# mitsuba-renderer/mitsuba2

Hardware: AMD Instinct MI355X
Metric: Msamples/sec (whole node), 1080p/512spp path integrator (higher is better)
Workload: dtype f32

## Files before the change

mitsuba2_amd/csrc/device/resident_kernel.h:

```cpp
#ifndef MIW_KERNEL
#define MIW_KERNEL __global__
#endif
MIW_KERNEL __launch_bounds__(MIW_BLOCK) void k_init_pixels(RenderParams P, U4 *st_out, uint32_t *pixel_out, InitArgs A) {
    uint32_t lane = blockIdx.x * blockDim.x + threadIdx.x;
    if (lane >= P.n_lanes) return;
    uint32_t tile = lane >> A.bs2_log2, i = lane & ((1u << A.bs2_log2) - 1u);
    uint32_t b = A.tile_list ? A.tile_list[tile] : tile;
    uint32_t bx = b % A.blocks_x, by = b / A.blocks_x;
    uint32_t x, y;
    morton_decode2(i, x, y);
    int32_t bw = P.film.crop_w - (int32_t) (bx * A.bs), bh = P.film.crop_h - (int32_t) (by * A.bs);
    if (bw > (int32_t) A.bs) bw = (int32_t) A.bs;
    if (bh > (int32_t) A.bs) bh = (int32_t) A.bs;
    if ((int32_t) x >= bw || (int32_t) y >= bh) {
        U4 st; st.x = st.y = 0; st.z = LF_DONE; st.w = 0;
        st_out[lane] = st; pixel_out[lane] = 0;
        return;
    }
    uint32_t px = (uint32_t) P.film.crop_x + bx * A.bs + x, py = (uint32_t) P.film.crop_y + by * A.bs + y;
    pixel_out[lane] = px | (py << 16);
    st_out[lane] = lane_seed_state(A.base_seed + (uint64_t) A.block_ids[b] * (uint64_t) (A.bs * A.bs) + i);
}

struct TileArgs {
    const uint32_t *tile_list; uint32_t blocks_x, bs, bs2_log2;
// ... 4 lines not shown
#ifndef MIW_PLACE_PIECES
#define MIW_PLACE_PIECES 4
#endif
template <bool Placed = true, bool Clock = false, bool Groups = false, bool Jobs = true, bool Frame = false>
struct QueueWork {
    static_assert(!Frame || (!Placed && !Groups && Jobs), "the frame twin: one queue of chunk jobs, no group counts");
    const LaneQueues *Q; uint32_t *next_pixel; uint32_t n_lanes, spp, lane, warn_negative;
    const FilmRec *film; const float *thr;
    uint32_t nq, per, q, dry, t_fetch;
    __device__ __forceinline__ void init_queues(uint32_t queues) {
        nq = Placed ? queues : 1u; per = nq > 1u ? MIW_PLACE_PIECES * 64u : n_lanes; q = 0u; dry = 0; t_fetch = 0;
        ticks = 0; quarter = 0; tail_prio = 0; sample_end_ = spp;
        if (Jobs) job_pend() = 0u;
        if (Placed && Q->simd_ids) {
            const uint32_t hw = (uint32_t) __builtin_amdgcn_s_getreg(4 | (0 << 6) | (31 << 11)),
                           xcc = (uint32_t) __builtin_amdgcn_s_getreg(20 | (0 << 6) | (3 << 11));
            const uint32_t key = ((xcc & 15u) << 10) | (((hw >> 13) & 7u) << 7) | (((hw >> 12) & 1u) << 6) | (((hw >> 8) & 15u) << 2) | ((hw >> 4) & 3u);
            if (nq > 1u) { const uint32_t id = Q->simd_ids[1u + key]; q = id < nq ? id : key % nq; }
            else if ((threadIdx.x & 63u) == 0u) Q->simd_ids[1u + key] = 1u;
        }
    }
    uint32_t ticks, quarter, tail_prio, sample_end_; uint32_t *prog;
    __device__ __forceinline__ void tick(uint32_t sample_idx, bool has_pixel) {
        if (Frame) return;
        if (!tail_prio) { ++ticks; return; }
        if ((uint32_t) __builtin_amdgcn_readfirstlane((int) ++ticks) & 15u) return;
        if (has_pixel) atomicMin(prog, sample_idx);
        const uint32_t v = *prog;
        *prog = 0xffffffffu;
        const uint32_t v4 = 4u * v, se = sample_end_;
        uint32_t qtr = v == 0xffffffffu ? 3u : (v4 >= se ? 1u : 0u) + (v4 >= 2u * se ? 1u : 0u) + (v4 >= 3u * se ? 1u : 0u);
        qtr = (uint32_t) __builtin_amdgcn_readfirstlane((int) qtr);
        if (qtr == quarter) return;
        quarter = qtr;
        if (qtr == 0u) __builtin_amdgcn_s_setprio(3); else if (qtr == 1u) __builtin_amdgcn_s_setprio(2);
        else if (qtr == 2u) __builtin_amdgcn_s_setprio(1); else __builtin_amdgcn_s_setprio(0);
    }
    __device__ __forceinline__ void enable_tail_prio(uint32_t sample_end, uint32_t *wave_word) {
        tail_prio = 1u; sample_end_ = sample_end; quarter = 0; prog = wave_word; *prog = 0xffffffffu; __builtin_amdgcn_s_setprio(3);
    }
    typedef uint32_t U4v __attribute__((ext_vector_type(4)));
    __device__ __forceinline__ static uint32_t &job_pend() { __shared__ uint32_t s_job_pend[MIW_BLOCK]; return s_job_pend[threadIdx.x & (MIW_BLOCK - 1)]; }
    __device__ __forceinline__ bool exhausted() const { return (!Frame && (!Jobs || !Q->job_chunk)) || job_pend() == 0xffffffffu; }
    __device__ __forceinline__ uint32_t job_end(uint32_t sample_idx, uint32_t sample_end) const {
        const uint32_t r = spp - sample_idx;
        return Jobs && (r & (r - 1u)) == 0u && r >= Q->job_min ? sample_idx : sample_end;
    }
    __device__ __forceinline__ bool fetch_job(uint32_t &pixel, U4 &st) {
        for (;;) {
            const uint32_t parked = job_pend();
            if (parked == 0xffffffffu) return false;
            uint32_t id = parked - 1u;
            const bool fresh = parked == 0u;
            const unsigned long long b = __ballot(fresh);
            if (fresh) {
                const uint32_t me = threadIdx.x & 63u, leader = (uint32_t) __ffsll((long long) b) - 1u;
                uint32_t base = 0;
                if (me == leader) base = atomicAdd(next_pixel, (uint32_t) __popcll(b));
                base = (uint32_t) __shfl((int) base, (int) leader, 64);
                id = base + __builtin_amdgcn_mbcnt_hi((uint32_t) (b >> 32), __builtin_amdgcn_mbcnt_lo((uint32_t) b, 0u));
                if (id >= Q->job_total) { job_pend() = 0xffffffffu; return false; }
            }
            const uint32_t j = id / n_lanes, slot = id - j * n_lanes;
            const uint32_t px = Q->pixel[slot];
            U4v w;
#if defined(__HIP_DEVICE_COMPILE__)
            asm volatile("global_load_dwordx4 %0, %1, off sc1\n\ts_waitcnt vmcnt(0)" : "=&v"(w) : "v"(Q->st + slot) : "memory");
#endif
            if (w.z & LF_DONE) { job_pend() = 0u; continue; }
            if (w.w != (j ? spp - (Q->job_pow >> (j - 1u)) : 0u)) { job_pend() = id + 1u; return false; }
            job_pend() = 0u;
            lane = slot; pixel = px;
            st.x = w.x; st.y = w.y; st.z = w.z; st.w = w.w;
            return true;
        }
    }
    __device__ __forceinline__ bool fetch(uint32_t &pixel, U4 &st) {
        if (Frame || (Jobs && Q->job_chunk)) return fetch_job(pixel, st);
        for (;;) {
            if (!Placed) {
                const unsigned long long b = __ballot(1);
                const uint32_t me = threadIdx.x & 63u, leader = (uint32_t) __ffsll((long long) b) - 1u;
                uint32_t base = 0;
                if (me == leader) base = atomicAdd(next_pixel, (uint32_t) __popcll(b));
                base = (uint32_t) __shfl((int) base, (int) leader, 64);
                const uint32_t l = base + __builtin_amdgcn_mbcnt_hi((uint32_t) (b >> 32), __builtin_amdgcn_mbcnt_lo((uint32_t) b, 0u));
                if (l >= n_lanes) return false;
                lane = l;
                st = Q->st[lane];
                if (st.z & LF_DONE) continue;
                pixel = Q->pixel[lane];
                return true;
            }
// ... 40 lines not shown
        }
        Q->st[lane] = st;
        if (Placed && Q->lane_cost) Q->lane_cost[lane] = cost_clock() - t_fetch + 1u;
        if (Groups && Q->group_done && (st.z & LF_DONE)) {
            __threadfence();
            const uint32_t g = lane >> Q->group_shift;
            if (atomicAdd(Q->group_done + g, 1u) + 1u == Q->group_expected[g]) {
                __threadfence_system();
                __hip_atomic_store(Q->group_flag + g, 1u, __ATOMIC_RELEASE, __HIP_MEMORY_SCOPE_SYSTEM);
            }
        }
    }
    __device__ __forceinline__ void put(uint32_t pixel, uint32_t sample_idx, V2 pos, const float *aovs) {
        if (Frame || Q->log_rec) {
            LogSink16<const float *> sink{ Q->log_rec, thr, film, lane, spp, Q->log_rej & 255u, Q->log_rej >> 8 };
            sink(pixel, sample_idx, pos, aovs);
        } else {
            LogSink sink; sink.log_pos = Q->log_pos; sink.log_val = Q->log_val; sink.lane = lane; sink.spp = spp; sink.warn_negative = warn_negative;
            sink(0u, sample_idx, pos, aovs);
        }
    }
};

#ifndef MIW_DIRECT_WAVES
#define MIW_DIRECT_WAVES 3
#endif
#ifndef MIW_PACKET_WAVES_ALL
#define MIW_PACKET_WAVES_ALL 4
#endif
#ifndef MIW_PACKET_WAVES
#define MIW_PACKET_WAVES 5
#endif
template <bool UseLog, int Tiny, int Mats = MATS_ALL, bool Analytic = (Tiny == 0), uint32_t Integ = INTEG_PATH, bool Groups = false, int Waves = 0, uint32_t Feat = FEAT_ALL>
__global__ __launch_bounds__(MIW_BLOCK, Waves ? Waves : Integ == INTEG_DIRECT ? MIW_DIRECT_WAVES : Tiny ? ((Mats == MATS_DIFFUSE && !MIW_SPECTRAL) ? (Tiny == 2 ? MIW_PACKET_WAVES : 4) : MIW_PACKET_WAVES_ALL) : MIW_TREE_WAVES) void k_path_resident(RenderParams P, SceneView sc, LaneQueues Q, double *accum, Counters *cnt,
                                                               TraceLds cfg, uint32_t sample_end, TileArgs T, uint32_t *next_pixel) {
    constexpr bool Frame = (Feat & FEAT_FRAME) != 0;
    static_assert(!Frame || (UseLog && Tiny != 0 && !Analytic && Integ == INTEG_PATH && !Groups && Waves == 0 && Feat == FEAT_FRAME), "a frame twin is the twin of a lean packet kernel");
    extern __shared__ uint4 smem[];
    stage_to_lds(sc, cfg, smem);
    const float *thr = stage_thresholds(smem, cfg, UseLog && (Frame || Q.log_rec) ? Q.log_thr : nullptr);
    constexpr bool Frames = MIW_LDS_TABLES && UseLog && Tiny != 0 && Integ != INTEG_DIRECT;
#if MIW_LDS_TABLES
    if constexpr (UseLog && Tiny != 0) stage_tables<true, mats_lights(Mats), mats_full(Mats), Frames>(sc, cfg, smem);
#endif
#if defined(MIW_SECTION_PROFILE) && defined(__HIP_DEVICE_COMPILE__)
    if ((threadIdx.x & 63u) == 0) { unsigned long long *b_ = miw_sec_buf(); for (int i = 0; i < 15; ++i) b_[i] = 0; b_[15] = __builtin_amdgcn_s_memtime(); }
// ... 3 lines not shown
    int tile_x0 = 0, tile_y0 = 0;
    if (!UseLog && T.side) {
        const uint32_t lane0 = blockIdx.x * blockDim.x, t = lane0 >> T.bs2_log2, q0 = lane0 & ((1u << T.bs2_log2) - 1u);
        const uint32_t b = T.tile_list ? T.tile_list[t] : t;
        uint32_t qx, qy;
        morton_decode2(q0, qx, qy);
        const int margin = (int) (T.side - 16u) / 2;
        tile_x0 = (int) ((b % T.blocks_x) * T.bs + qx) - margin;
        tile_y0 = (int) ((b / T.blocks_x) * T.bs + qy) - margin;
        for (uint32_t i = threadIdx.x; i < T.side * T.side * MIW_FILM_CHANNELS; i += blockDim.x) tile[i] = 0.0;
        __syncthreads();
    }
    LaneCounters local; local.segments = local.samples = local.shadow_rays = 0;
    auto tr2 = [&](V3 o, float mint, V3 dE, float maxtE, bool hasE, V3 dS, float maxtS, bool hasS, F4 &hE, bool &occS) {
        trace2<Tiny, Analytic, Integ != INTEG_DIRECT, Frame>(sc, cfg, smem, o, mint, dE, maxtE, hasE, dS, maxtS, hasS, hE, occS);
    };
    if (UseLog) {
        QueueWork<Tiny != 0 && !Frame, false, Groups, true, Frame> work; work.Q = &Q; work.next_pixel = next_pixel; work.n_lanes = P.n_lanes; work.spp = P.spp; work.lane = 0; work.warn_negative = P.film.warn_negative;
        work.film = &P.film; work.thr = thr; work.init_queues(cfg.queues ? cfg.queues : 1u);
        if constexpr (!Frame) {
            __shared__ uint32_t s_prog[MIW_BLOCK / 64];
            if (cfg.tail_prio) work.enable_tail_prio(sample_end, &s_prog[threadIdx.x >> 6]);
        }
        if constexpr (Integ == INTEG_DIRECT) pixel_stream_render_direct<Mats, Analytic>(P, sc, sample_end, work, tr2, &local);
        else pixel_stream_render<Mats, Analytic, Frames, Feat & FEAT_ALL>(P, sc, sample_end, work, tr2, &local);
    } else if (lane < P.n_lanes) {
        U4 st = Q.st[lane];
        if (!(st.z & LF_DONE)) {
            const uint32_t pixel = Q.pixel[lane];
            if (T.side) {
                TileAdd add; add.tile = tile; add.x0 = tile_x0; add.y0 = tile_y0; add.side = (int) T.side;
                SplatXYSink<TileAdd> sink; sink.film = &P.film; sink.add = add;
                st = pixel_render<Integ, mats_nested(Mats) ? Mats : MATS_ALL>(P, sc, pixel, st, sample_end, tr2, sink, &local);
            } else {
                FilmAdd add; add.accum = accum;
                SplatSink<FilmAdd> sink; sink.film = &P.film; sink.add = add;
                st = pixel_render<Integ, mats_nested(Mats) ? Mats : MATS_ALL>(P, sc, pixel, st, sample_end, tr2, sink, &local);
            }
            Q.st[lane] = st;
        }
    }
    if (!UseLog && T.side) {
        __syncthreads();
        const int n = (int) (T.side * T.side);
        for (int i = (int) threadIdx.x; i < n * MIW_FILM_CHANNELS; i += (int) blockDim.x) {
            const double v = tile[i];
            if (v == 0.0) continue;
            const int texel = i / MIW_FILM_CHANNELS, k = i - texel * MIW_FILM_CHANNELS;
            const int fx = tile_x0 + texel % (int) T.side, fy = tile_y0 + texel / (int) T.side;
            unsafeAtomicAdd(accum + ((size_t) fy * P.film.crop_w + fx) * MIW_FILM_CHANNELS + k, v);
        }
    }
    unsigned long long a = wave_sum(local.segments), b = wave_sum(local.samples), c = wave_sum(local.shadow_rays);
    if ((threadIdx.x & 63) == 0) {
        Counters *shard = cnt + ((blockIdx.x * (MIW_BLOCK / 64) + (threadIdx.x >> 6)) & (MIW_CNT_SHARDS - 1));
        if (a) atomicAdd(&shard->segments, a);
        if (b) atomicAdd(&shard->samples, b);
        if (c) atomicAdd(&shard->shadow_rays, c);
#if defined(MIW_SECTION_PROFILE) && defined(__HIP_DEVICE_COMPILE__)
        { unsigned long long *b_ = miw_sec_buf(); for (int i = 0; i < 15; ++i) if (b_[i]) atomicAdd(&g_sections[i], b_[i]); }
#endif
    }
}
```

mitsuba2_amd/csrc/miwave.hip:

```cpp
#include <hip/hip_runtime.h>
#include <stdio.h>
#include <stdlib.h>
#include <string.h>
#include <stdarg.h>
#include <string>
#include <vector>
#include <chrono>
#include <atomic>
#include <cmath>
#include <map>
#include <string>
#include <algorithm>

#include "../../include/miwave.h"
#include "kernel_pick.h"
#if defined(MIW_CLASS_PART) || defined(MIW_AOV_UNIT)
#define MIW_KERNELS_ONLY 1
#endif
#if defined(MIW_SECTION_PROFILE)
__device__ unsigned long long g_sections[16];
#endif
#if defined(MIW_PHASE_STATS)
__device__ unsigned long long g_phase_stats[15];
#endif
// ... 116 lines not shown
    { "MIW_MAX_LEAF", "host SAH builder: triangles per leaf" },
    { "MIW_NO_STACK", "1: no LDS-stack walk (stackless BVH2 walk, wavefront plan)" },
    { "MIW_BVH4", "0: no 4-wide tree (the phase machine steps through the BVH2)" },
    { "MIW_BVH4_FAN", "2 | 3 | 4: widest node the 4-wide collapse may build" },
    { "MIW_BVH4_HOST", "1: the 4-wide tree is collapsed on the host from the read-back BVH2" },
    { "MIW_BVH8", "0: mi_bvh_build skips the 8-wide tree / mi_render keeps the 4-wide walk" },
    { "MIW_STACK8_FULL", "1: the 8-wide walk keeps the 16-entry LDS column instead of one entry per tree level" },
    { "MIW_ENV_TOP", "0: the environment warp's top levels are not staged in LDS" },
    { "MIW_PHASED", "0: tree scenes take the lock-step kernel instead of the phase machine" },
    { "MIW_PHASED_WAVES", "3 | 4: wavefronts per SIMD the phase machine is launched for" },
    { "MIW_TRIO", "0: MATS_PLAIN kernels where the MATS_TRIO class would do" },
    { "MIW_SHADE_VOTE", "num:den of the phase machine's shade vote" },
    { "MIW_LOOP_EXIT", "node:triangle hand-over ratios of the phase machine's walk loops" },
    { "MIW_POOLED", "1: tree scenes take k_path_pooled (walk jobs pooled across the workgroup; experimental, slower: DESIGN.md)" },
    { "MIW_POOL_SHAPE", "12x1 | 8x2: wavefronts per workgroup x pixels per lane of k_path_pooled" },
    { "MIW_POOL_VOTE", "shade_min:walk_min:node_min:tri_min:claim_min of k_path_pooled" },
    { "MIW_TAIL_PRIO", "0: no least-progress-first wave priorities; 1: also in a packet kernel's launch of chunk jobs, which runs without them by default (and then keeps its lean kernel instead of the frame twin)" },
    { "MIW_WG_PER_CU", "workgroups per CU of the packet kernels' persistent grid" },
    { "MIW_PLACE", "0: shards of about one pixel per lane skip the measuring launch + placed queues" },
    { "MIW_JOB_CHUNK", "smallest chunk of a full frame's pixel jobs, in samples (a power of two; default 64, the phase machine 32): the pixels' sample streams are cut into halving chunks drawn chunk-major from one queue; 0: a job = all the samples of a pixel" },
    { "MIW_JOB_CHUNK_FORCE", "1: chunk jobs whatever the frame's size (tests of the hand-over between lanes)" },
    { "MIW_LEAN", "0: a packet scene without environment map and vertex normals, rendered without the moment integrator, keeps the full path kernel instead of its lean twin (kernel_pick.h: packet_features)" },
    { "MIW_FRAME_TWIN", "0: a full frame of chunk jobs keeps the lean twin of its packet path kernel instead of the frame twin, which has the facts of such a launch compiled in (kernel_pick.h: frame_twin)" },
    { "MIW_PACKET_SHARD4", "0: a plain-diffuse packet job of at most four wavefronts of pixels per SIMD keeps the five-wavefront (96-register) kernel" },
    { "MIW_PLACE_MEASURE", "divisor: the measuring launch runs spp / divisor samples" },
    { "MIW_PLACE_SPREAD", "0 | 1: placed pieces = consecutive sorted lanes | one lane of every cost stratum" },
    { "MIW_STREAM", "0: plan 1 walks with one kernel per list slice instead of the persistent stream kernel" },
    { "MIW_FILM_LEGACY", "1: the 24-byte position log + k_film_blocks for every filter" },
    { "MIW_FILM_LANES", "0 | 1 | 2: k_film_lanes off / over the tile-interleaved log / over [lane][sample]" },
    { "MIW_FILM_CHAINS", "0: the replay over the tile-interleaved log runs k_film_lanes (a wavefront per block position) instead of k_film_chains (a wavefront per chain of positions of equal weight)" },
    { "MIW_FILM_CHAINS_U", "4 | 8: records in flight per lane of k_film_chains: 8 (the default) compiled for two wavefronts per SIMD, 4 for three" },
    { "MIW_FILM_QUADS", "0 | 24 | 28 | 42 | 44: k_film_quads group shape (0: off)" },
    { "MIW_FILM_COLUMNS", "0 | 42 | 44 | 82: k_film_columns group shape" },
    { "MIW_FILM_GROUP", "2 | 3 | 4: k_film_groups group shape" },
    { "MIW_FL_NT", "0: k_film_lanes reads the log with plain instead of streaming loads" },
    { "MIW_FILM_OVERLAP", "1: part of the film replay of a full Cornell-class frame is queued on three more streams beside the path kernel, sets of 64-tile groups each behind the flags their last pixels raise (default 0: measured +0 - 1 %); 2: without the waits (timing probe: the film is the previous frame's)" },
    { "MIW_FILM_OVERLAP_SET", "groups of 64 tiles per launch of that replay (default 4)" },
    { "MIW_FILM_OVERLAP_ROOM", "workgroups the path kernel's grid is short of filling the device while the replay runs beside it (default 32: one per CU on 32 CUs)" },
    { "MIW_FILM_OVERLAP_LEAN", "0: the launches of that replay are the 168-register kernel (default 1: the 128-register form)" },
    { "MIW_FILM_OVERLAP_BESIDE", "groups of 64 tiles replayed beside the path kernel; the rest in one launch after it (default: three quarters)" },
    { "MIW_FILM_OVERLAP_PRIO", "s_setprio of the replay wavefronts that run beside the path kernel, 0 .. 3 (default 0)" },
    { "MIW_FQ_U", "2 | 4 | 8: records per trip of k_film_quads" },
    { "MIW_RCCL", "0: mi_film_reduce never uses RCCL (device add)" },
    { "MIW_RCCL_FORCE", "1: mi_film_reduce takes the RCCL branch for one context too (tests)" }
};
struct Options {
// ... 1758 lines not shown
static bool out_of_time(const RenderFrame &F) {
    return F.cfg->timeout_s > 0.f &&
           std::chrono::duration<double>(std::chrono::steady_clock::now() - F.wall0).count() > F.cfg->timeout_s;
}
static SceneView view_over_tree8(const mi_ctx *c) {
    SceneView v = c->view;
    v.nodes8 = c->d_nodes8.p; v.tris = c->d_tris8.p; if (v.tri_vn) v.tri_vn = c->d_tri_vn8.p;
    return v;
}
static InitArgs init_args(const RenderFrame &F) {
    InitArgs A; A.block_ids = F.c->d_block_ids.p; A.tile_list = F.cfg->tile_list ? F.c->d_tile_list.p : nullptr;
    A.blocks_x = F.blocks_x; A.blocks_y = F.blocks_y; A.bs = F.bs; A.bs2_log2 = F.bs2_log2; A.base_seed = F.cfg->base_seed;
    return A;
}

struct PathRoute {
    bool direct, tiny;
    uint32_t n_simd, per_launch;
    bool phased, phased_placeable, phased8; int ph_waves;
    bool packet_shard4; uint32_t feat, res_waves;
    bool place; uint32_t measure_end, n_pieces;
    int overlap_mode; bool overlap;
    bool pooled;
};
static mi_status path_route(RenderFrame &F, const miw_pick::Facts &facts, const RenderLds &L, PathRoute &R) {
    mi_ctx *c = F.c; const mi_render_cfg *cfg = F.cfg; const Options &ropt = F.ropt; const FilmPlan &FP = F.FP;
    const int film_mode = FP.film_mode; const uint32_t n_lanes = F.n_lanes, n_tiles = F.n_tiles;
    const bool direct = F.P.integrator == INTEG_DIRECT, tables_fit = L.lay.tables_fit; const size_t rlds = L.lay.rlds;
    const uint32_t n_simd = (uint32_t) c->cu_count * 4u;
    const uint32_t per_launch = cfg->samples_per_launch > 0 ? (uint32_t) cfg->samples_per_launch : 128u;
    const bool tiny = facts.tiny;
    const bool phased_on = !ropt.off("MIW_PHASED");
    const bool trio_kernel = miw_pick::trio_kernel(facts);
    const bool phased = phased_on && !direct && !tiny && c->lds_cfg.stack && (c->view.nodes4 != nullptr || trio_kernel) && (tables_fit || !MIW_LDS_TABLES);
    const int ph_waves = ropt.num("MIW_PHASED_WAVES", 4) == 4 ? 4 : 3;
    const bool phased_placeable = phased && c->view.nodes4 != nullptr && ph_waves == 4;
    const bool phased8 = phased_placeable && L.walk8;
    if (L.stack8_sized && !phased8) return fail(c, MI_ERR_STATE, "render: the LDS stack was sized for the 8-wide walk, which this launch does not run");
    bool packet_shard4 = !phased && tiny && c->diffuse_only && !MIW_SPECTRAL && !direct && c->view.tri_count <= 32u && MIW_PACKET_WAVES > 4 && film_mode == 1 && n_lanes <= 64u * 4u * n_simd;
    if (ropt.off("MIW_PACKET_SHARD4")) packet_shard4 = false;
    const uint32_t feat = miw_pick::packet_features_kernel(miw_pick::packet_features(c->have_env, c->shape_normals, c->emitter_normals, cfg->moment_pass != 0), !ropt.off("MIW_LEAN"));
    const uint32_t res_waves_compiled = miw_plan::res_waves_compiled(phased, (uint32_t) ph_waves, tiny, c->diffuse_only && !MIW_SPECTRAL, c->view.tri_count <= 32u, packet_shard4,
                                                                     (uint32_t) MIW_TREE_WAVES, (uint32_t) MIW_PACKET_WAVES, (uint32_t) MIW_PACKET_WAVES_ALL);
    const uint32_t res_waves = tiny && film_mode == 1 ? std::max(1u, std::min(res_waves_compiled, miw_plan::lds_workgroups(rlds))) : res_waves_compiled;
    bool place = film_mode == 1 && !direct && (tiny || phased_placeable) && miw_plan::place_window(n_lanes, res_waves, n_simd) &&
                 cfg->spp >= 128u && per_launch >= cfg->spp && cfg->timeout_s <= 0.f;
    if (ropt.off("MIW_PLACE")) place = false;
    uint32_t measure_div = (uint32_t) std::max(2, ropt.num("MIW_PLACE_MEASURE", 8));
    const uint32_t measure_end = place ? std::max<uint32_t>(16u, cfg->spp / measure_div) : 0u;
    const uint32_t n_pieces = (n_lanes + 63u) / 64u;
    const int overlap_mode = ropt.num("MIW_FILM_OVERLAP", 0);
    const bool overlap = overlap_mode != 0 && c->overlap_state != 0 && film_mode == 1 && FP.rec16 && FP.film_lanes != 0 && FP.log_il != 0 && !place && !phased  && tiny && c->diffuse_only && !MIW_SPECTRAL && !direct  &&
                         per_launch >= cfg->spp && cfg->timeout_s <= 0.f && n_tiles > 0;
#if MIW_SPECTRAL
    const bool pooled = false;
#else
    const bool pooled = phased8 && !place && L.pooled_fits;
#endif
    R.direct = direct; R.tiny = tiny; R.n_simd = n_simd; R.per_launch = per_launch;
    R.phased = phased; R.phased_placeable = phased_placeable; R.phased8 = phased8; R.ph_waves = ph_waves;
    R.packet_shard4 = packet_shard4; R.feat = feat; R.res_waves = res_waves;
    R.place = place; R.measure_end = measure_end; R.n_pieces = n_pieces;
    R.overlap_mode = overlap_mode; R.overlap = overlap; R.pooled = pooled;
    return MI_OK;
}

static mi_status place_prepare(RenderFrame &F, const PathRoute &R, size_t &place_tmp_bytes) {
// ... 45 lines not shown
        HIP_TRY(c, hipStreamSynchronize(s));
        if (first_lane < n_lanes) HIP_TRY(c, hipMemcpy(&px, c->q_pixel.p + first_lane, sizeof(uint32_t), hipMemcpyDeviceToHost));
        double csum = 0.0; uint32_t with = 0;
        for (uint32_t v : all) if (v) { csum += (double) v; ++with; }
        K.place_cost_max = all.empty() ? 0u : all[0]; K.place_cost_mean = with ? csum / with : 0.0; K.place_max_pixel = px;
        K.place_cost_unit = phased ? 1u : 0u; K.place_measure_spp = measure_end;
    }
    if (K.placed && ropt.get("MIW_DEBUG")) {
        std::vector<uint32_t> cur(n_simd), ids(1u + (1u << 14)), cost(n_pieces);
        (void) hipMemcpy(cur.data(), c->d_next_pixel.p, n_simd * sizeof(uint32_t), hipMemcpyDeviceToHost);
        (void) hipMemcpy(ids.data(), c->d_simd_ids.p, ids.size() * sizeof(uint32_t), hipMemcpyDeviceToHost);
        (void) hipMemcpy2D(cost.data(), sizeof(uint32_t), c->d_cost_sorted.p, Q.piece_a * sizeof(uint32_t), sizeof(uint32_t), n_pieces, hipMemcpyDeviceToHost);
        uint32_t keys = 0, key_or = 0, full = 0, over = 0; uint64_t csum = 0; uint32_t cmin = ~0u, cmax = 0;
        for (uint32_t k = 0; k < (1u << 14); ++k) if (ids[1 + k] != 0xffffffffu) { ++keys; key_or |= k; }
        ids[0] = keys;
        for (uint32_t v : cur) { full += v >= 64u * MIW_PLACE_PIECES; over += v > 64u * MIW_PLACE_PIECES; }
        for (uint32_t v : cost) { csum += v; cmin = std::min(cmin, v); cmax = std::max(cmax, v); }
        fprintf(stderr, "[miwave] placed queues: %u SIMDs numbered, %u distinct hardware keys (bits used 0x%x), %u of %u queues drained (%u asked beyond their end), "
                        "cost of the dearest pixel of a piece min / mean / max = %u / %.0f / %u (iterations, or 256-cycle units)\n", ids[0], keys, key_or, full, n_simd, over, cmin, (double) csum / n_pieces, cmax);
    }
    return MI_OK;
}

static void chunk_jobs(RenderFrame &F, const PathRoute &R, const RenderLds &L, uint32_t done) {
    const mi_render_cfg *cfg = F.cfg; const Options &ropt = F.ropt; LaneQueues &Q = F.Q; mi_counters &K = F.K; const uint32_t n_lanes = F.n_lanes;
    const bool tiny = R.tiny, phased = R.phased, place = R.place, overlap = R.overlap, pooled_fits = L.pooled_fits;
    const uint32_t per_launch = R.per_launch, res_waves = R.res_waves, n_simd = R.n_simd;
    Q.job_chunk = Q.job_pow = Q.job_total = 0u; Q.job_min = 0x80000000u;
    if ((tiny || (phased && MIW_PHASED_JOBS != 0)) && !pooled_fits && !place && !overlap && done == 0 && per_launch >= cfg->spp && cfg->timeout_s <= 0.f) {
        uint32_t jmin = tiny ? 64u : 32u;
        if (const char *e = ropt.get("MIW_JOB_CHUNK")) jmin = (uint32_t) std::max(0, atoi(e));
        bool enough = miw_plan::chunks_enough(n_lanes, res_waves, n_simd);
        if (ropt.on("MIW_JOB_CHUNK_FORCE")) enough = true;
        const miw_plan::ChunkSchedule cs = miw_plan::chunk_schedule(cfg->spp, jmin);
        if (cs.job_min && enough && cs.chunks >= 2u && (uint64_t) n_lanes * cs.chunks < (1ull << 31)) {
            Q.job_chunk = cs.job_min; Q.job_min = cs.job_min; Q.job_pow = cs.job_pow; Q.job_total = (uint32_t) ((uint64_t) n_lanes * cs.chunks);
            K.job_chunk = cs.job_min; K.job_chunks = (uint32_t) cs.chunks;
        }
    }
}

struct PathLaunch {
    dim3 grid;
    TraceLds rcfg;
    SceneView view8;
    TileArgs TA; size_t tile_bytes = 0;
    uint32_t end = 0;
    uint32_t feat_launched = FEAT_ALL;
    bool frame_launched = false;
};
static mi_status atomic_film_tile(RenderFrame &F, const InitArgs &A, PathLaunch &PK) {
    mi_ctx *c = F.c; const mi_render_cfg *cfg = F.cfg; const int film_mode = F.FP.film_mode; const uint32_t bs = F.bs, blocks_x = F.blocks_x, bs2_log2 = F.bs2_log2;
    TileArgs &TA = PK.TA; size_t &tile_bytes = PK.tile_bytes;
// ... 68 lines not shown
#define MIW_PHASED_PICKED(M, A, WV, W, PL) if (pick.mats == (M) && pick.analytic == (A) && ph_waves == (WV) && wide == (W) && place == (PL)) MIW_PHASED_LAUNCH_(M, A, WV, W, PL); else
            MIW_PHASED_LIST(MIW_PHASED_PICKED) return fail(c, MI_ERR_STATE, "render: no k_path_phased<%d, %d, ., %d, %d, %d> in the library", pick.mats, (int) pick.analytic, ph_waves, wide, (int) place);
#undef MIW_PHASED_PICKED
        }
#undef MIW_PHASED_LAUNCH
#undef MIW_PHASED_LAUNCH_
#define MIW_PACKET_SPECIAL(...) MIW_TIMED(6, MIW_LAUNCH_NAMED(ropt, (__VA_ARGS__), pgrid, block, rlds, s, P, c->view, Q, (double *) nullptr, c->d_cnt.p, rcfg, end, TA, c->d_next_pixel.p))
        else if (Q.group_done && c->view.tri_count <= 32u)
            MIW_PACKET_SPECIAL(k_path_resident<true, 2, MATS_DIFFUSE, false, INTEG_PATH, true>);
        else if (Q.group_done)
            MIW_PACKET_SPECIAL(k_path_resident<true, 1, MATS_DIFFUSE, false, INTEG_PATH, true>);
        else if (packet_shard4 && !Q.group_done && feat == FEAT_NONE) {
            feat_launched = FEAT_NONE;
            MIW_PACKET_SPECIAL(k_path_resident<true, 2, MATS_DIFFUSE, false, INTEG_PATH, false, 4, FEAT_NONE>);
        }
        else if (packet_shard4 && !Q.group_done)
            MIW_PACKET_SPECIAL(k_path_resident<true, 2, MATS_DIFFUSE, false, INTEG_PATH, false, 4>);
#undef MIW_PACKET_SPECIAL
        else {
            const miw_pick::Pick pick = direct ? miw_pick::resident_direct(facts) : miw_pick::resident_path(facts, false);
            miw_pick::LaunchFacts lf;
            lf.job_chunks = Q.job_chunk != 0u; lf.log_rec16 = Q.log_rec != nullptr; lf.one_queue = rcfg.queues == 1u; lf.tail_prio = rcfg.tail_prio != 0u;
            lf.leaf_filter = c->lds_cfg.leaves != 0u; lf.group_counts = Q.group_done != nullptr;
            const bool frame = miw_pick::frame_twin(pick, direct, feat, lf, !ropt.off("MIW_FRAME_TWIN"));
#define MIW_FRAME_LAUNCH(T, M) if (frame && MIW_PICKED(T, M, false)) { feat_launched = FEAT_NONE; frame_launched = true; MIW_TIMED(6, MIW_LAUNCH_NAMED(ropt, (k_path_resident<true, T, M, false, INTEG_PATH, false, 0, FEAT_FRAME>), pgrid, block, rlds, s, P, c->view, Q, (double *) nullptr, c->d_cnt.p, rcfg, end, TA, c->d_next_pixel.p)); } else
            MIW_LEAN_LIST(MIW_FRAME_LAUNCH)
#undef MIW_FRAME_LAUNCH
#define MIW_LEAN_LAUNCH(T, M) if (feat == FEAT_NONE && !direct && MIW_PICKED(T, M, false)) { feat_launched = FEAT_NONE; MIW_TIMED(6, MIW_LAUNCH_NAMED(ropt, (k_path_resident<true, T, M, false, INTEG_PATH, false, 0, FEAT_NONE>), pgrid, block, rlds, s, P, c->view, Q, (double *) nullptr, c->d_cnt.p, rcfg, end, TA, c->d_next_pixel.p)); } else
            MIW_LEAN_LIST(MIW_LEAN_LAUNCH)
#undef MIW_LEAN_LAUNCH
#define MIW_RESIDENT_LAUNCH(T, M, A, I) if (integ == (I) && MIW_PICKED(T, M, A)) MIW_TIMED(6, MIW_LAUNCH_NAMED(ropt, (k_path_resident<true, T, M, A, I>), pgrid, block, (T) != 0 ? rlds : rlds_plain, s, P, c->view, Q, (double *) nullptr, c->d_cnt.p, rcfg, end, TA, c->d_next_pixel.p)); else
            MIW_RESIDENT_LIST(MIW_RESIDENT_LAUNCH) return fail(c, MI_ERR_STATE, "render: no k_path_resident<true, %d, %d, %d, %u> in the library", pick.tiny, pick.mats, (int) pick.analytic, integ);
#undef MIW_RESIDENT_LAUNCH
        }
    } else {
        const miw_pick::Pick pick = miw_pick::resident_atomic(facts);
#define MIW_ATOMIC_LAUNCH(T, M, A, I) if (integ == (I) && MIW_PICKED(T, M, A)) MIW_TIMED(6, MIW_LAUNCH_NAMED(ropt, (k_path_resident<false, T, M, A, I>), grid, block, c->lds_bytes + tile_bytes, s, P, c->view, Q, c->d_accum.p, c->d_cnt.p, c->lds_cfg, end, TA, (uint32_t *) nullptr)); else
        MIW_ATOMIC_LIST(MIW_ATOMIC_LAUNCH) return fail(c, MI_ERR_STATE, "render: no k_path_resident<false, %d, %d, %d, %u> in the library", pick.tiny, pick.mats, (int) pick.analytic, integ);
#undef MIW_ATOMIC_LAUNCH
    }
    return MI_OK;
}

static mi_status render_resident(RenderFrame &F, const miw_pick::Facts &facts, const RenderLds &L, FilmReplay &replay, mi_status &result) {
    mi_ctx *c = F.c; const mi_render_cfg *cfg = F.cfg; const Options &ropt = F.ropt; const RenderParams &P = F.P; hipStream_t s = F.s;
    LaneQueues &Q = F.Q; LaunchTimer &T = F.T; mi_counters &K = F.K; const int film_mode = F.FP.film_mode;
    PathLaunch PK; PK.grid = dim3((F.n_lanes + MIW_BLOCK - 1) / MIW_BLOCK);
    const InitArgs A = init_args(F);
// ... 1 lines not shown
    HIP_TRY(c, hipGetLastError());
    PathRoute R;
    MI_TRY(path_route(F, facts, L, R));
    HIP_TRY(c, c->d_next_pixel.resize(std::max<uint32_t>(8u, R.n_simd)));
    PK.rcfg = L.lay.cfg;
    PK.view8 = R.phased8 ? view_over_tree8(c) : c->view;
    size_t place_tmp_bytes = 0;
    if (R.place) MI_TRY(place_prepare(F, R, place_tmp_bytes));
    MI_TRY(atomic_film_tile(F, A, PK));
    const uint32_t sync_every = 8;
    uint32_t launches = 0;
    bool place_stats_due = false;
    for (uint32_t done = 0; done < cfg->spp; ) {
        PK.end = cfg->spp - done < R.per_launch ? cfg->spp : done + R.per_launch;
        PK.feat_launched = FEAT_ALL; PK.frame_launched = false;
        if (film_mode == 1) {
            HIP_TRY(c, hipMemsetAsync(c->d_next_pixel.p, 0, c->d_next_pixel.n * sizeof(uint32_t), s));
            PK.rcfg.queues = 1u; Q.lane_cost = nullptr; Q.lane_sorted = nullptr; Q.piece_list = nullptr; Q.simd_ids = nullptr;
            if (R.overlap && done == 0) {
                MI_TRY(film_replay_setup(F, replay));
                MI_TRY(overlap_prepare(F));
                if (Q.group_done) HIP_TRY(c, hipEventRecord(c->ev_fork, s));
            }
            chunk_jobs(F, R, L, done);
            if (R.place && done == 0) { PK.end = R.measure_end; Q.lane_cost = c->d_lane_cost.p; Q.simd_ids = c->d_simd_ids.p; }
            else if (R.place) MI_TRY(place_deal(F, R, place_tmp_bytes, PK.rcfg, place_stats_due));
        }
        MI_TRY(launch_path_kernel(F, facts, R, L, PK));
        if (Q.group_done) {
            MI_TRY(overlap_enqueue(F, replay, R.overlap_mode != 2));
            if (c->replay_enqueued) { K.film_overlapped = 1u; K.film_groups = c->replay_launches; }
            Q.group_done = nullptr; Q.group_expected = nullptr; Q.group_flag = nullptr;
        }
        if (ropt.get("MIW_DEBUG") && R.tiny && !R.phased) fprintf(stderr, "[miwave] packet path kernel launched: scene features 0x%x of 0x%x compiled in (mask chosen for the render: 0x%x)\n", PK.feat_launched, (uint32_t) FEAT_ALL, R.feat);
        if (ropt.get("MIW_DEBUG") && R.tiny && !R.phased) fprintf(stderr, "[miwave] packet path kernel launched: frame twin %s\n", PK.frame_launched ? "yes (chunk jobs, one queue, 16-byte log, no tail priorities, leaf filter compiled in)" : "no");
        K.n_path++; K.iterations++;
        done = PK.end;
        if ((++launches % sync_every == 0 || cfg->timeout_s > 0.f || c->cancel.load()) && done < cfg->spp) {
            HIP_TRY(c, hipGetLastError());
            HIP_TRY(c, hipStreamSynchronize(s));
            T.drain();
            if (c->cancel.load() || out_of_time(F)) { result = MI_ERR_CANCELLED; break; }
        }
    }
    HIP_TRY(c, hipGetLastError());
    Counters sum;
    MI_TRY(read_counters(F, sum));
    MI_TRY(place_statistics(F, R, place_stats_due));
    print_debug_statistics(c, ropt, K);
    T.drain();
    return MI_OK;
}

#if !MIW_SPECTRAL
static mi_status render_wavefront(RenderFrame &F, mi_status &result) {
    mi_ctx *c = F.c; const Options &ropt = F.ropt; const RenderParams &P = F.P; hipStream_t s = F.s;
    const LaneQueues &Q = F.Q; LaunchTimer &T = F.T; mi_counters &K = F.K; const int film_mode = F.FP.film_mode; const uint32_t n_lanes = F.n_lanes;
    dim3 grid((n_lanes + MIW_BLOCK - 1) / MIW_BLOCK), block(MIW_BLOCK);
// ... 149 lines not shown
```

mitsuba2_amd/csrc/render_plan.h:

```cpp
#pragma once
#include <algorithm>
#include <cstddef>
#include <cstdint>
#include <vector>

#define MIW_LDS_PER_CU (160u * 1024u)
#define MIW_LDS_PER_WORKGROUP (MIW_LDS_PER_CU / 4u)
#define MIW_LDS_STATIC 1024u
#define MIW_LDS_GRANULE 512u

namespace miw_plan {

struct ChunkSchedule { uint32_t job_min, job_pow; uint64_t chunks; };
inline ChunkSchedule chunk_schedule(uint32_t spp, uint32_t jmin) {
    jmin = (jmin & (jmin - 1u)) ? 0u : jmin;
    uint32_t pow2 = 1u;
    while (pow2 * 2u < spp) pow2 *= 2u;
    uint64_t chunks = 1u;
    for (uint32_t r = pow2; jmin && r >= jmin && r < spp; r >>= 1) ++chunks;
    return { jmin, pow2, chunks };
}
inline bool chunks_enough(uint32_t n_lanes, uint32_t res_waves, uint32_t n_simd) { return (uint64_t) n_lanes * 5u >= (uint64_t) 6u * 64u * res_waves * n_simd; }

inline uint32_t deal_pieces(uint32_t n_pieces, uint32_t nqueues, uint32_t slots, std::vector<uint32_t> &list) {
    if (nqueues < 2u || (uint64_t) nqueues * slots < n_pieces) return 0u;
    list.assign((size_t) nqueues * slots, 0xffffffffu);
    for (uint32_t i = 0; i < n_pieces; ++i) {
        const uint32_t round = i / nqueues, k = i % nqueues, qd = (round & 1u) ? nqueues - 1u - k : k;
        list[(size_t) qd * slots + round] = i;
    }
    return nqueues;
}

inline uint32_t lds_workgroups(size_t dyn) {
    const size_t per = (dyn + MIW_LDS_STATIC + 16u + MIW_LDS_GRANULE - 1u) / MIW_LDS_GRANULE * MIW_LDS_GRANULE;
    return (uint32_t) (MIW_LDS_PER_CU / per);
}

inline unsigned persistent_wg_per_cu(bool direct, unsigned res_waves) { return std::max(4u, direct ? 4u : res_waves); }
inline unsigned persistent_grid(unsigned grid_x, unsigned cu_count, unsigned wg_per_cu, unsigned room, unsigned resident_waves) {
    const unsigned resident = cu_count * resident_waves;
    const unsigned full = room ? std::min(cu_count * wg_per_cu, resident) : cu_count * wg_per_cu;
    return std::min<unsigned>(grid_x, full > 2u * room ? full - room : full);
}

// ... 8 lines not shown
```

Before: 5094.

## Batch chunk-job draws per wavefront into an LDS ring in the frame twin

In the frame-twin path kernel, each wavefront now claims a batch of up to 32 chunk-job ids with one atomic and prefetches their state and pixel words into a per-wave LDS ring during tick(). Later fetches take ids from that pool and skip the global atomic and the uncached global load unless the pooled state is stale. Per-thread counters are replaced by wave-level LDS ds_add_u64 counters, the smallest chunk drops to 16 when the twin is taken, and the twin launch reserves a fixed 26 KB of LDS. Prefetched state can go stale before use, in which case it falls back to a global reload, and the larger LDS footprint may lower occupancy.

```diff
diff --git a/mitsuba2_amd/csrc/device/resident_kernel.h b/mitsuba2_amd/csrc/device/resident_kernel.h
--- a/mitsuba2_amd/csrc/device/resident_kernel.h
+++ b/mitsuba2_amd/csrc/device/resident_kernel.h
@@ -1,6 +1,7 @@
 #ifndef MIW_KERNEL
 #define MIW_KERNEL __global__
 #endif
+#include "../render_plan.h"
 MIW_KERNEL __launch_bounds__(MIW_BLOCK) void k_init_pixels(RenderParams P, U4 *st_out, uint32_t *pixel_out, InitArgs A) {
     uint32_t lane = blockIdx.x * blockDim.x + threadIdx.x;
     if (lane >= P.n_lanes) return;
@@ -51,7 +52,7 @@
     }
     uint32_t ticks, quarter, tail_prio, sample_end_; uint32_t *prog;
     __device__ __forceinline__ void tick(uint32_t sample_idx, bool has_pixel) {
-        if (Frame) return;
+        if (Frame) { refill(); return; }
         if (!tail_prio) { ++ticks; return; }
         if ((uint32_t) __builtin_amdgcn_readfirstlane((int) ++ticks) & 15u) return;
         if (has_pixel) atomicMin(prog, sample_idx);
@@ -75,14 +76,65 @@
         const uint32_t r = spp - sample_idx;
         return Jobs && (r & (r - 1u)) == 0u && r >= Q->job_min ? sample_idx : sample_end;
     }
+    __device__ __forceinline__ uint32_t pool_size() const { return (uint32_t) __builtin_amdgcn_readfirstlane((int) lds_get(wave_words() + 2)); }
+    __device__ __forceinline__ static uint32_t *wave_words() { extern __shared__ uint4 smem_pool[]; return reinterpret_cast<uint32_t *>(smem_pool) + MIW_POOL_AT / 4u + (threadIdx.x >> 6) * (MIW_POOL_STRIDE / 4u); }
+    __device__ __forceinline__ static uint32_t *ring_state(uint32_t id) { return wave_words() + MIW_POOL_HEAD / 4u + 4u * miw_plan::pool_ring_slot(id, MIW_POOL_MAX); }
+    __device__ __forceinline__ static uint32_t *ring_pixel(uint32_t id) { return wave_words() + MIW_POOL_HEAD / 4u + 4u * MIW_POOL_MAX + miw_plan::pool_ring_slot(id, MIW_POOL_MAX); }
+    __device__ __forceinline__ static uint32_t lds_get(const uint32_t *p) { return __hip_atomic_load(p, __ATOMIC_RELAXED, __HIP_MEMORY_SCOPE_WAVEFRONT); }
+    __device__ __forceinline__ static void lds_set(uint32_t *p, uint32_t v) { __hip_atomic_store(p, v, __ATOMIC_RELAXED, __HIP_MEMORY_SCOPE_WAVEFRONT); }
+    __device__ __forceinline__ void init_pool(uint32_t pool_) {
+        uint32_t *wv = wave_words();
+        if ((threadIdx.x & 63u) < MIW_POOL_HEAD / 4u) lds_set(wv + (threadIdx.x & 63u), (threadIdx.x & 63u) == 2u ? pool_ : 0u);
+    }
+    __device__ __forceinline__ uint32_t chunk_first(uint32_t j) const { return j ? spp - (Q->job_pow >> (j - 1u)) : 0u; }
+    __device__ __forceinline__ static U4v load_state(const U4 *p) {
+        U4v w;
+#if defined(__HIP_DEVICE_COMPILE__)
+        asm volatile("global_load_dwordx4 %0, %1, off sc1\n\ts_waitcnt vmcnt(0)" : "=&v"(w) : "v"(p) : "memory");
+#endif
+        return w;
+    }
+    __device__ __forceinline__ void refill() {
+        const uint32_t pool = pool_size();
+        if (!pool) return;
+        uint32_t *wv = wave_words();
+        miw_plan::JobCursor cur{ (uint32_t) __builtin_amdgcn_readfirstlane((int) lds_get(wv)), (uint32_t) __builtin_amdgcn_readfirstlane((int) lds_get(wv + 1)) };
+        if (!miw_plan::pool_empty(cur) || miw_plan::pool_dry(cur)) return;
+        const unsigned long long m = __ballot(1);
+        const uint32_t rank = __builtin_amdgcn_mbcnt_hi((uint32_t) (m >> 32), __builtin_amdgcn_mbcnt_lo((uint32_t) m, 0u)), n_run = (uint32_t) __popcll(m);
+        uint32_t base = 0;
+        if (rank == 0u) base = atomicAdd(next_pixel, pool);
+        base = (uint32_t) __builtin_amdgcn_readfirstlane((int) base);
+        cur = miw_plan::pool_batch(base, pool, Q->job_total);
+        if (!miw_plan::pool_dry(cur)) for (uint32_t id = base + rank; id < cur.end; id += n_run) {
+            const uint32_t j = id / n_lanes, slot = id - j * n_lanes;
+            const uint32_t px = Q->pixel[slot];
+            const U4v w = load_state(Q->st + slot);
+            uint32_t *e = ring_state(id);
+            lds_set(e, w.x); lds_set(e + 1, w.y); lds_set(e + 2, w.z); lds_set(e + 3, w.w);
+            lds_set(ring_pixel(id), px);
+        }
+        if (rank == 0u) { lds_set(wv, cur.next); lds_set(wv + 1, cur.end); }
+    }
     __device__ __forceinline__ bool fetch_job(uint32_t &pixel, U4 &st) {
         for (;;) {
             const uint32_t parked = job_pend();
             if (parked == 0xffffffffu) return false;
             uint32_t id = parked - 1u;
             const bool fresh = parked == 0u;
-            const unsigned long long b = __ballot(fresh);
-            if (fresh) {
+            bool draw = fresh, pooled = false;
+            if constexpr (Frame) {
+                const unsigned long long a = __ballot(fresh);
+                uint32_t *wv = wave_words();
+                const miw_plan::JobCursor cur{ lds_get(wv), lds_get(wv + 1) };
+                const uint32_t rank = __builtin_amdgcn_mbcnt_hi((uint32_t) (a >> 32), __builtin_amdgcn_mbcnt_lo((uint32_t) a, 0u)), asking = (uint32_t) __popcll(a);
+                if (fresh && rank == 0u) lds_set(wv, miw_plan::pool_after(cur, asking).next);
+                if (fresh && miw_plan::pool_dry(cur)) { job_pend() = 0xffffffffu; return false; }
+                pooled = fresh && rank < miw_plan::pool_take(cur, asking);
+                id = pooled ? cur.next + rank : id; draw = fresh && !pooled;
+            }
+            const unsigned long long b = __ballot(draw);
+            if (draw) {
                 const uint32_t me = threadIdx.x & 63u, leader = (uint32_t) __ffsll((long long) b) - 1u;
                 uint32_t base = 0;
                 if (me == leader) base = atomicAdd(next_pixel, (uint32_t) __popcll(b));
@@ -91,13 +143,18 @@
                 if (id >= Q->job_total) { job_pend() = 0xffffffffu; return false; }
             }
             const uint32_t j = id / n_lanes, slot = id - j * n_lanes;
-            const uint32_t px = Q->pixel[slot];
+            uint32_t px = 0;
             U4v w;
-#if defined(__HIP_DEVICE_COMPILE__)
-            asm volatile("global_load_dwordx4 %0, %1, off sc1\n\ts_waitcnt vmcnt(0)" : "=&v"(w) : "v"(Q->st + slot) : "memory");
-#endif
+            bool have = false;
+            if (Frame && pooled) {
+                const uint32_t *e = ring_state(id);
+                w.x = lds_get(e); w.y = lds_get(e + 1); w.z = lds_get(e + 2); w.w = lds_get(e + 3);
+                px = lds_get(ring_pixel(id));
+                have = (w.z & LF_DONE) || w.w == chunk_first(j);
+            }
+            if (!have) { px = Q->pixel[slot]; w = load_state(Q->st + slot); }
             if (w.z & LF_DONE) { job_pend() = 0u; continue; }
-            if (w.w != (j ? spp - (Q->job_pow >> (j - 1u)) : 0u)) { job_pend() = id + 1u; return false; }
+            if (w.w != chunk_first(j)) { job_pend() = id + 1u; return false; }
             job_pend() = 0u;
             lane = slot; pixel = px;
             st.x = w.x; st.y = w.y; st.z = w.z; st.w = w.w;
@@ -184,6 +241,22 @@
     }
 };
 
+template <uint32_t K> struct WaveCount {
+    __device__ __forceinline__ static uint32_t *block() { extern __shared__ uint4 smem_cnt[]; return reinterpret_cast<uint32_t *>(smem_cnt) + MIW_POOL_AT / 4u + (threadIdx.x >> 6) * (MIW_POOL_STRIDE / 4u); }
+    __device__ __forceinline__ static unsigned long long *word() { return reinterpret_cast<unsigned long long *>(block() + K); }
+    __device__ __forceinline__ void operator++(int) const {
+#if defined(__HIP_DEVICE_COMPILE__)
+        unsigned long long keep, sum;
+        asm volatile("s_mov_b64 %0, exec\n\ts_bcnt1_i32_b64 vcc_lo, exec\n\ts_ff1_i32_b64 vcc_hi, exec\n\ts_lshl_b64 exec, 1, vcc_hi\n\ts_mov_b32 vcc_hi, 0\n\t"
+                     "v_mov_b64 %1, vcc\n\tds_add_u64 %2, %1 offset:%3\n\ts_mov_b64 exec, %0"
+                     : "=&s"(keep), "=&v"(sum) : "v"((uint32_t) (uintptr_t) block()), "n"(4u * K) : "memory", "scc", "vcc");
+#endif
+    }
+    __device__ __forceinline__ unsigned long long get() const { return __hip_atomic_load(word(), __ATOMIC_RELAXED, __HIP_MEMORY_SCOPE_WAVEFRONT); }
+};
+static_assert(MIW_BLOCK / 64u * MIW_POOL_STRIDE == MIW_POOL_FRONT, "a block per wavefront of the workgroup, found by threadIdx.x >> 6");
+struct WaveCounters { WaveCount<4u> segments; WaveCount<6u> samples; WaveCount<8u> shadow_rays; };
+
 #ifndef MIW_DIRECT_WAVES
 #define MIW_DIRECT_WAVES 3
 #endif
@@ -233,6 +306,11 @@
             __shared__ uint32_t s_prog[MIW_BLOCK / 64];
             if (cfg.tail_prio) work.enable_tail_prio(sample_end, &s_prog[threadIdx.x >> 6]);
         }
+        if constexpr (Frame) {
+            work.init_pool(T.side);
+            const WaveCounters wave{};
+            pixel_stream_render<Mats, Analytic, Frames, Feat & FEAT_ALL>(P, sc, sample_end, work, tr2, &wave);
+        } else
         if constexpr (Integ == INTEG_DIRECT) pixel_stream_render_direct<Mats, Analytic>(P, sc, sample_end, work, tr2, &local);
         else pixel_stream_render<Mats, Analytic, Frames, Feat & FEAT_ALL>(P, sc, sample_end, work, tr2, &local);
     } else if (lane < P.n_lanes) {
@@ -262,7 +340,10 @@
             unsafeAtomicAdd(accum + ((size_t) fy * P.film.crop_w + fx) * MIW_FILM_CHANNELS + k, v);
         }
     }
-    unsigned long long a = wave_sum(local.segments), b = wave_sum(local.samples), c = wave_sum(local.shadow_rays);
+    unsigned long long a, b, c;
+    if constexpr (Frame) {
+        a = WaveCount<4u>{}.get(); b = WaveCount<6u>{}.get(); c = WaveCount<8u>{}.get();
+    } else { a = wave_sum(local.segments); b = wave_sum(local.samples); c = wave_sum(local.shadow_rays); }
     if ((threadIdx.x & 63) == 0) {
         Counters *shard = cnt + ((blockIdx.x * (MIW_BLOCK / 64) + (threadIdx.x >> 6)) & (MIW_CNT_SHARDS - 1));
         if (a) atomicAdd(&shard->segments, a);
diff --git a/mitsuba2_amd/csrc/miwave.hip b/mitsuba2_amd/csrc/miwave.hip
--- a/mitsuba2_amd/csrc/miwave.hip
+++ b/mitsuba2_amd/csrc/miwave.hip
@@ -162,6 +162,7 @@
     { "MIW_JOB_CHUNK_FORCE", "1: chunk jobs whatever the frame's size (tests of the hand-over between lanes)" },
     { "MIW_LEAN", "0: a packet scene without environment map and vertex normals, rendered without the moment integrator, keeps the full path kernel instead of its lean twin (kernel_pick.h: packet_features)" },
     { "MIW_FRAME_TWIN", "0: a full frame of chunk jobs keeps the lean twin of its packet path kernel instead of the frame twin, which has the facts of such a launch compiled in (kernel_pick.h: frame_twin)" },
+    { "MIW_JOB_POOL", "chunk-job ids a wavefront of a frame twin draws from the queue at a time, their state words read into its LDS block with the draw (a power of two from 2 to 32; default 32); 0: every job drawn on its own (resident_kernel.h: QueueWork::refill)" },
     { "MIW_PACKET_SHARD4", "0: a plain-diffuse packet job of at most four wavefronts of pixels per SIMD keeps the five-wavefront (96-register) kernel" },
     { "MIW_PLACE_MEASURE", "divisor: the measuring launch runs spp / divisor samples" },
     { "MIW_PLACE_SPREAD", "0 | 1: placed pieces = consecutive sorted lanes | one lane of every cost stratum" },
@@ -1966,6 +1967,7 @@
     bool place; uint32_t measure_end, n_pieces;
     int overlap_mode; bool overlap;
     bool pooled;
+    bool twin_fits; uint32_t job_pool; size_t twin_rlds;
 };
 static mi_status path_route(RenderFrame &F, const miw_pick::Facts &facts, const RenderLds &L, PathRoute &R) {
     mi_ctx *c = F.c; const mi_render_cfg *cfg = F.cfg; const Options &ropt = F.ropt; const FilmPlan &FP = F.FP;
@@ -1987,6 +1989,9 @@
     const uint32_t res_waves_compiled = miw_plan::res_waves_compiled(phased, (uint32_t) ph_waves, tiny, c->diffuse_only && !MIW_SPECTRAL, c->view.tri_count <= 32u, packet_shard4,
                                                                      (uint32_t) MIW_TREE_WAVES, (uint32_t) MIW_PACKET_WAVES, (uint32_t) MIW_PACKET_WAVES_ALL);
     const uint32_t res_waves = tiny && film_mode == 1 ? std::max(1u, std::min(res_waves_compiled, miw_plan::lds_workgroups(rlds))) : res_waves_compiled;
+    R.job_pool = miw_plan::pool_size(ropt.num("MIW_JOB_POOL", 32));
+    R.twin_fits = tiny && film_mode == 1 && rlds <= MIW_POOL_AT && std::min(res_waves_compiled, miw_plan::lds_workgroups(MIW_TWIN_LDS)) >= res_waves;
+    R.twin_rlds = MIW_TWIN_LDS;
     bool place = film_mode == 1 && !direct && (tiny || phased_placeable) && miw_plan::place_window(n_lanes, res_waves, n_simd) &&
                  cfg->spp >= 128u && per_launch >= cfg->spp && cfg->timeout_s <= 0.f;
     if (ropt.off("MIW_PLACE")) place = false;
@@ -2078,13 +2083,22 @@
     return MI_OK;
 }
 
-static void chunk_jobs(RenderFrame &F, const PathRoute &R, const RenderLds &L, uint32_t done) {
+static bool takes_frame_twin(const Options &ropt, const miw_pick::Pick &pick, bool direct, uint32_t feat, const miw_pick::LaunchFacts &lf) {
+    return miw_pick::frame_twin(pick, direct, feat, lf, !ropt.off("MIW_FRAME_TWIN"));
+}
+static void chunk_jobs(RenderFrame &F, const miw_pick::Facts &facts, const PathRoute &R, const RenderLds &L, uint32_t done) {
     const mi_render_cfg *cfg = F.cfg; const Options &ropt = F.ropt; LaneQueues &Q = F.Q; mi_counters &K = F.K; const uint32_t n_lanes = F.n_lanes;
     const bool tiny = R.tiny, phased = R.phased, place = R.place, overlap = R.overlap, pooled_fits = L.pooled_fits;
     const uint32_t per_launch = R.per_launch, res_waves = R.res_waves, n_simd = R.n_simd;
     Q.job_chunk = Q.job_pow = Q.job_total = 0u; Q.job_min = 0x80000000u;
     if ((tiny || (phased && MIW_PHASED_JOBS != 0)) && !pooled_fits && !place && !overlap && done == 0 && per_launch >= cfg->spp && cfg->timeout_s <= 0.f) {
         uint32_t jmin = tiny ? 64u : 32u;
+        if (tiny && R.twin_fits && R.job_pool && miw_plan::chunks_enough(n_lanes, res_waves, n_simd)) {
+            miw_pick::LaunchFacts lf;
+            lf.job_chunks = true; lf.log_rec16 = Q.log_rec != nullptr; lf.one_queue = true; lf.tail_prio = ropt.on("MIW_TAIL_PRIO");
+            lf.leaf_filter = F.c->lds_cfg.leaves != 0u; lf.group_counts = false;
+            if (takes_frame_twin(ropt, miw_pick::resident_path(facts, false), R.direct, R.feat, lf)) jmin = 16u;
+        }
         if (const char *e = ropt.get("MIW_JOB_CHUNK")) jmin = (uint32_t) std::max(0, atoi(e));
         bool enough = miw_plan::chunks_enough(n_lanes, res_waves, n_simd);
         if (ropt.on("MIW_JOB_CHUNK_FORCE")) enough = true;
@@ -2199,8 +2213,9 @@
             miw_pick::LaunchFacts lf;
             lf.job_chunks = Q.job_chunk != 0u; lf.log_rec16 = Q.log_rec != nullptr; lf.one_queue = rcfg.queues == 1u; lf.tail_prio = rcfg.tail_prio != 0u;
             lf.leaf_filter = c->lds_cfg.leaves != 0u; lf.group_counts = Q.group_done != nullptr;
-            const bool frame = miw_pick::frame_twin(pick, direct, feat, lf, !ropt.off("MIW_FRAME_TWIN"));
-#define MIW_FRAME_LAUNCH(T, M) if (frame && MIW_PICKED(T, M, false)) { feat_launched = FEAT_NONE; frame_launched = true; MIW_TIMED(6, MIW_LAUNCH_NAMED(ropt, (k_path_resident<true, T, M, false, INTEG_PATH, false, 0, FEAT_FRAME>), pgrid, block, rlds, s, P, c->view, Q, (double *) nullptr, c->d_cnt.p, rcfg, end, TA, c->d_next_pixel.p)); } else
+            const bool frame = R.twin_fits && takes_frame_twin(ropt, pick, direct, feat, lf);
+            TileArgs TW = TA; TW.side = R.job_pool;
+#define MIW_FRAME_LAUNCH(T, M) if (frame && MIW_PICKED(T, M, false)) { feat_launched = FEAT_NONE; frame_launched = true; MIW_TIMED(6, MIW_LAUNCH_NAMED(ropt, (k_path_resident<true, T, M, false, INTEG_PATH, false, 0, FEAT_FRAME>), pgrid, block, R.twin_rlds, s, P, c->view, Q, (double *) nullptr, c->d_cnt.p, rcfg, end, TW, c->d_next_pixel.p)); } else
             MIW_LEAN_LIST(MIW_FRAME_LAUNCH)
 #undef MIW_FRAME_LAUNCH
 #define MIW_LEAN_LAUNCH(T, M) if (feat == FEAT_NONE && !direct && MIW_PICKED(T, M, false)) { feat_launched = FEAT_NONE; MIW_TIMED(6, MIW_LAUNCH_NAMED(ropt, (k_path_resident<true, T, M, false, INTEG_PATH, false, 0, FEAT_NONE>), pgrid, block, rlds, s, P, c->view, Q, (double *) nullptr, c->d_cnt.p, rcfg, end, TA, c->d_next_pixel.p)); } else
@@ -2248,7 +2263,7 @@
                 MI_TRY(overlap_prepare(F));
                 if (Q.group_done) HIP_TRY(c, hipEventRecord(c->ev_fork, s));
             }
-            chunk_jobs(F, R, L, done);
+            chunk_jobs(F, facts, R, L, done);
             if (R.place && done == 0) { PK.end = R.measure_end; Q.lane_cost = c->d_lane_cost.p; Q.simd_ids = c->d_simd_ids.p; }
             else if (R.place) MI_TRY(place_deal(F, R, place_tmp_bytes, PK.rcfg, place_stats_due));
         }
@@ -2259,7 +2274,8 @@
             Q.group_done = nullptr; Q.group_expected = nullptr; Q.group_flag = nullptr;
         }
         if (ropt.get("MIW_DEBUG") && R.tiny && !R.phased) fprintf(stderr, "[miwave] packet path kernel launched: scene features 0x%x of 0x%x compiled in (mask chosen for the render: 0x%x)\n", PK.feat_launched, (uint32_t) FEAT_ALL, R.feat);
-        if (ropt.get("MIW_DEBUG") && R.tiny && !R.phased) fprintf(stderr, "[miwave] packet path kernel launched: frame twin %s\n", PK.frame_launched ? "yes (chunk jobs, one queue, 16-byte log, no tail priorities, leaf filter compiled in)" : "no");
+        if (ropt.get("MIW_DEBUG") && R.tiny && !R.phased && !PK.frame_launched) fprintf(stderr, "[miwave] packet path kernel launched: frame twin no\n");
+        if (ropt.get("MIW_DEBUG") && R.tiny && !R.phased && PK.frame_launched) fprintf(stderr, "[miwave] packet path kernel launched: frame twin yes (chunk jobs, one queue, 16-byte log, no tail priorities, leaf filter compiled in), job pool %u, smallest chunk %u, %zu bytes of LDS per workgroup\n", R.job_pool, Q.job_min, R.twin_rlds);
         K.n_path++; K.iterations++;
         done = PK.end;
         if ((++launches % sync_every == 0 || cfg->timeout_s > 0.f || c->cancel.load()) && done < cfg->spp) {
diff --git a/mitsuba2_amd/csrc/render_plan.h b/mitsuba2_amd/csrc/render_plan.h
--- a/mitsuba2_amd/csrc/render_plan.h
+++ b/mitsuba2_amd/csrc/render_plan.h
@@ -21,6 +21,27 @@
     return { jmin, pow2, chunks };
 }
 inline bool chunks_enough(uint32_t n_lanes, uint32_t res_waves, uint32_t n_simd) { return (uint64_t) n_lanes * 5u >= (uint64_t) 6u * 64u * res_waves * n_simd; }
+
+struct JobCursor { uint32_t next, end; };
+#define MIW_POOL_DRY 0xffffffffu
+constexpr uint32_t pool_size(int given) { return given >= 2 && given <= 32 && (given & (given - 1)) == 0 ? (uint32_t) given : 0u; }
+constexpr JobCursor pool_batch(uint32_t base, uint32_t pool, uint32_t job_total) {
+    return base >= job_total ? JobCursor{ MIW_POOL_DRY, MIW_POOL_DRY } : JobCursor{ base, job_total - base < pool ? job_total : base + pool };
+}
+constexpr bool pool_dry(JobCursor c) { return c.next == MIW_POOL_DRY; }
+constexpr bool pool_empty(JobCursor c) { return c.next == c.end; }
+constexpr uint32_t pool_take(JobCursor c, uint32_t asking) { return pool_dry(c) ? 0u : (c.end - c.next < asking ? c.end - c.next : asking); }
+constexpr JobCursor pool_after(JobCursor c, uint32_t asking) { return JobCursor{ c.next + pool_take(c, asking), c.end }; }
+constexpr uint32_t pool_ring_slot(uint32_t id, uint32_t pool) { return id & (pool - 1u); }
+#define MIW_POOL_HEAD 48u
+constexpr uint32_t pool_wave_bytes(uint32_t pool) { return MIW_POOL_HEAD + 20u * pool; }
+constexpr uint32_t pool_lds_bytes(uint32_t pool, uint32_t waves_per_workgroup) { return waves_per_workgroup * pool_wave_bytes(pool); }
+#define MIW_POOL_MAX 32u
+#define MIW_POOL_STRIDE 688u
+#define MIW_POOL_FRONT 2752u
+#define MIW_TWIN_LDS 26624u
+#define MIW_POOL_AT (MIW_TWIN_LDS - MIW_POOL_FRONT)
+static_assert(pool_wave_bytes(MIW_POOL_MAX) == MIW_POOL_STRIDE && pool_lds_bytes(MIW_POOL_MAX, 4u) == MIW_POOL_FRONT && MIW_POOL_FRONT % 16u == 0u && MIW_TWIN_LDS % 16u == 0u, "the twin's blocks");
 
 inline uint32_t deal_pieces(uint32_t n_pieces, uint32_t nqueues, uint32_t slots, std::vector<uint32_t> &list) {
     if (nqueues < 2u || (uint64_t) nqueues * slots < n_pieces) return 0u;
```

Result: faster. 5154 (median of 6 runs) (+1.2%).
